# jstmn/cppflow

Hardware: AMD Instinct MI355X
Metric: LM-IK iterations/sec (seeds x waypoints) (higher is better)
Workload: dtype f32

## Files before the change

cppflow_amd/build.py:

```python

import os
import subprocess
import sys

_HERE = os.path.dirname(os.path.abspath(__file__))
CSRC = os.path.join(_HERE, "csrc")
SOURCES = ["cppflow_hip.hip", "fused_static.hip"]
EXTRA_FLAGS = {"fused_static.hip": ["-O2", "-mllvm", "-amdgpu-sched-strategy=max-ilp", "-mllvm", "-enable-post-misched=0"]}
HEADERS = ["lmik_device.h", "obstacle_reach.h", "robots_gen.h", "rtc_specialize.h", "kernels_chain.h", "kernels_collision.h", "kernels_fused.h", "kernels_track.h", "kernels_quad.h", "kernels_eval.h",
           "kernels_coupled.h", "kernels_dp.h", "kernels_optloop.h", "kernels_scene.h", "kernels_motion.h", "kernels_motion_resolve.h", os.path.join("..", "..", "include", "cppflow_hip.h"),
           os.path.join("..", "..", "include", "cppflow_hip_debug.h")]
OUT = os.path.join(CSRC, "libcppflow_hip.so")

HIPCC_FLAGS = [
    "--offload-arch=gfx950",
    "-O3",
    "-std=c++17",
    "-fPIC",
    "-ffp-contract=off",
    "-fhip-fp32-correctly-rounded-divide-sqrt",
    "-fno-slp-vectorize",
    "-Wno-comment",
]


def source_hash() -> str:
    import hashlib

    h = hashlib.sha256()
    for name in SOURCES + [n for n in HEADERS if n != "rtc_specialize.h"] + ["rtc_specialize.h"]:
        with open(os.path.join(CSRC, name), "rb") as f:
            h.update(name.encode() + b"\0" + f.read() + b"\0")
    h.update(" ".join(HIPCC_FLAGS).encode())
    for name in SOURCES:
        h.update((name + " " + " ".join(EXTRA_FLAGS.get(name, []))).encode())
    h.update(" ".join(link_flags()).encode())
    return h.hexdigest()[:32]


def link_flags():
    return [f for f in HIPCC_FLAGS if f.startswith("--offload-arch=") or f == "-fPIC"] + ["-shared"]


def built_id() -> str:
    if not os.path.exists(OUT):
        return ""
    import re

    with open(OUT, "rb") as f:
        m = re.search(rb"CPPF_BUILD_ID=([0-9a-f]{32})", f.read())
    return m.group(1).decode() if m else ""


def needs_build() -> bool:
    if not os.path.exists(OUT):
        return True
    return built_id() != source_hash()


EMBEDDED = ["lmik_device.h", "kernels_chain.h", "kernels_collision.h", "kernels_fused.h", "kernels_track.h", "kernels_quad.h"]
EMBEDDED_OUT = os.path.join(CSRC, "embedded_src.inc")


def write_embedded_sources() -> bool:
    parts = ["// embedded_src.inc -- GENERATED by cppflow_amd/build.py (the device headers as strings for hipRTC); do not edit."]
    files = [(n, os.path.join(CSRC, n)) for n in EMBEDDED] + [("../../include/cppflow_hip.h", os.path.join(CSRC, "..", "..", "include", "cppflow_hip.h"))]
    parts.append(f"static const int kEmbeddedCount = {len(files)};")
    parts.append("static const char* const kEmbeddedNames[] = {" + ", ".join(f'"{n}"' for n, _ in files) + "};")
    parts.append("static const char* const kEmbeddedSources[] = {")
    for _, path in files:
        text = open(path).read()
        assert ')CPPFSRC"' not in text
        chunks = [text[i : i + 12000] for i in range(0, len(text), 12000)]
        parts.append("    " + "\n    ".join(f'R"CPPFSRC({c})CPPFSRC"' for c in chunks) + ",")
    parts.append("};")
    out = "\n".join(parts) + "\n"
    if os.path.exists(EMBEDDED_OUT) and open(EMBEDDED_OUT).read() == out:
        return False
    with open(EMBEDDED_OUT, "w") as f:
        f.write(out)
    return True


def build(force: bool = False, verbose: bool = False) -> str:
    from cppflow_amd import gen_robots

    if gen_robots.write() and verbose:
        print("regenerated", gen_robots.OUT)
    if write_embedded_sources() and verbose:
        print("regenerated", EMBEDDED_OUT)
    if not force and not needs_build():
        return OUT
    hipcc = os.environ.get("HIPCC", "hipcc")
    objdir = os.path.join(CSRC, "obj")
    os.makedirs(objdir, exist_ok=True)
    procs, objs = [], []
    for src in SOURCES:
        obj = os.path.join(objdir, os.path.splitext(src)[0] + ".o")
        cmd = [hipcc] + HIPCC_FLAGS + EXTRA_FLAGS.get(src, []) + [f'-DCPPF_BUILD_ID="{source_hash()}"', "-c", "-o", obj, os.path.join(CSRC, src)]
        if verbose:
            print(" ".join(cmd))
        procs.append((cmd, subprocess.Popen(cmd, cwd=CSRC)))
        objs.append(obj)
    failed = None
    for cmd, p in procs:
        if p.wait() != 0 and failed is None:
            failed = (p.returncode, cmd)
            for _, other in procs:
                if other.poll() is None:
                    other.kill()
    if failed is not None:
        raise subprocess.CalledProcessError(*failed)
    cmd = [hipcc] + link_flags() + ["-o", OUT] + objs
    if verbose:
        print(" ".join(cmd))
    subprocess.run(cmd, check=True, cwd=CSRC)
    return OUT


TEST_SRC = os.path.join(_HERE, "..", "tests", "native", "rcp_sweep.hip")
TEST_OUT = os.path.join(_HERE, "..", "tests", "native", "libcppf_testkernels.so")


def build_test_kernels(force: bool = False, verbose: bool = False) -> str:
    deps = [TEST_SRC, os.path.join(CSRC, "lmik_device.h"), os.path.abspath(__file__)]
    if not force and os.path.exists(TEST_OUT) and all(os.path.getmtime(TEST_OUT) >= os.path.getmtime(d) for d in deps):
        return TEST_OUT
    cmd = [os.environ.get("HIPCC", "hipcc")] + HIPCC_FLAGS + ["-shared", "-o", TEST_OUT, TEST_SRC]
    if verbose:
        print(" ".join(cmd))
    subprocess.run(cmd, check=True)
    return TEST_OUT


if __name__ == "__main__":
    print(build(force="--force" in sys.argv, verbose=True))
    print(build_test_kernels(force="--force" in sys.argv, verbose=True))
```

Baseline: 80.88 billion.

## Post-process fused_static assembly with VGPR bank reassignment tool

Changes the build for fused_static.hip so it compiles to device assembly first. A custom tool (tools/vgpr_banks) then rewrites the assembly, presumably remapping VGPRs to cut register-bank conflicts. The rewritten file is assembled, linked, bundled and embedded into the host object. This aims to remove bank-conflict stalls in the hot fused kernel, at the cost of a fragile multi-step toolchain and the risk of bugs in the assembly rewriter.

```diff
diff --git a/cppflow_amd/build.py b/cppflow_amd/build.py
--- a/cppflow_amd/build.py
+++ b/cppflow_amd/build.py
@@ -11,6 +11,11 @@
            "kernels_coupled.h", "kernels_dp.h", "kernels_optloop.h", "kernels_scene.h", "kernels_motion.h", "kernels_motion_resolve.h", os.path.join("..", "..", "include", "cppflow_hip.h"),
            os.path.join("..", "..", "include", "cppflow_hip_debug.h")]
 OUT = os.path.join(CSRC, "libcppflow_hip.so")
+BANKED = ["fused_static.hip"]
+BANKS_TOOL_SRC = os.path.join("tools", "vgpr_banks.cpp")
+BANKS_TOOL_FLAGS = ["-std=c++17", "-O2"]
+LLVM_BIN = os.environ.get("CPPF_LLVM_BIN", "/opt/rocm/lib/llvm/bin")
+DEVICE_TARGET = "hipv4-amdgcn-amd-amdhsa--gfx950"
 
 HIPCC_FLAGS = [
     "--offload-arch=gfx950",
@@ -35,7 +40,45 @@
     for name in SOURCES:
         h.update((name + " " + " ".join(EXTRA_FLAGS.get(name, []))).encode())
     h.update(" ".join(link_flags()).encode())
+    with open(os.path.join(CSRC, BANKS_TOOL_SRC), "rb") as f:
+        h.update(BANKS_TOOL_SRC.encode() + b"\0" + f.read() + b"\0")
+    h.update(" ".join(BANKS_TOOL_FLAGS).encode())
+    for name in BANKED:
+        for step in banked_commands(name, "", ""):
+            h.update(" ".join(os.path.basename(a) for a in step).encode() + b"\0")
     return h.hexdigest()[:32]
+
+
+def vgpr_banks_enabled() -> bool:
+    return os.environ.get("CPPF_VGPR_BANKS", "1") != "0"
+
+
+def banked_commands(src: str, objdir: str, build_id: str):
+    stem = os.path.join(objdir, os.path.splitext(src)[0])
+    hipcc = os.environ.get("HIPCC", "hipcc")
+    common = [hipcc] + HIPCC_FLAGS + EXTRA_FLAGS.get(src, []) + [f'-DCPPF_BUILD_ID="{build_id}"']
+    asm = stem + ".s"
+    steps = [common + ["--cuda-device-only", "-S", "-o", asm, os.path.join(CSRC, src)]]
+    if vgpr_banks_enabled():
+        steps.append([os.path.join(objdir, "vgpr_banks"), asm, "-o", stem + ".banks.s"])
+        asm = stem + ".banks.s"
+    steps += [
+        [os.path.join(LLVM_BIN, "clang"), "-x", "assembler", "-target", "amdgcn-amd-amdhsa", "-mcpu=gfx950", "-c", "-o", stem + ".dev.o", asm],
+        [os.path.join(LLVM_BIN, "ld.lld"), "-m", "elf64_amdgpu", "--no-undefined", "-shared", "-o", stem + ".co", stem + ".dev.o"],
+        [os.path.join(LLVM_BIN, "clang-offload-bundler"), "-type=o", "-bundle-align=4096", f"-targets=host-x86_64-unknown-linux-gnu,{DEVICE_TARGET}",
+         "-input=/dev/null", "-input=" + stem + ".co", "-output=" + stem + ".hipfb"],
+        common + ["--cuda-host-only", "-Xclang", "-fcuda-include-gpubinary", "-Xclang", stem + ".hipfb", "-c", "-o", stem + ".o", os.path.join(CSRC, src)],
+    ]
+    return steps
+
+
+def build_banks_tool(objdir: str, verbose: bool = False) -> str:
+    exe = os.path.join(objdir, "vgpr_banks")
+    cmd = [os.environ.get("CXX") or os.path.join(LLVM_BIN, "clang++")] + BANKS_TOOL_FLAGS + ["-o", exe, os.path.join(CSRC, BANKS_TOOL_SRC)]
+    if verbose:
+        print(" ".join(cmd))
+    subprocess.run(cmd, check=True)
+    return exe
 
 
 def link_flags():
@@ -97,12 +140,26 @@
     procs, objs = [], []
     for src in SOURCES:
         obj = os.path.join(objdir, os.path.splitext(src)[0] + ".o")
+        objs.append(obj)
+        if src in BANKED:
+            continue
         cmd = [hipcc] + HIPCC_FLAGS + EXTRA_FLAGS.get(src, []) + [f'-DCPPF_BUILD_ID="{source_hash()}"', "-c", "-o", obj, os.path.join(CSRC, src)]
         if verbose:
             print(" ".join(cmd))
         procs.append((cmd, subprocess.Popen(cmd, cwd=CSRC)))
-        objs.append(obj)
     failed = None
+    try:
+        if vgpr_banks_enabled():
+            build_banks_tool(objdir, verbose)
+        for src in BANKED:
+            for cmd in banked_commands(src, objdir, source_hash()):
+                if verbose:
+                    print(" ".join(cmd))
+                subprocess.run(cmd, check=True, cwd=CSRC)
+    except (subprocess.CalledProcessError, OSError) as e:
+        failed = (getattr(e, "returncode", 127), getattr(e, "cmd", str(e)))
+        for _, other in procs:
+            other.kill()
     for cmd, p in procs:
         if p.wait() != 0 and failed is None:
             failed = (p.returncode, cmd)
```

After: 80.95 billion, median of 3. No clear change (+0.1%).
